# QiaoK/MPI-Asynchronous-Communication-Test

Measured on AMD Instinct MI355X. Metric: aggregate exchange GB/s + max total time, all-to-many/many-to-all, 1–8 GPUs, higher is better.
Workload: dtype u8

## Files before the change

### include/xg.h

```cpp
#ifndef XG_H
#define XG_H

#include <stddef.h>
#include <stdint.h>

#include "xg_sched.h"

#ifdef __cplusplus
extern "C" {
#endif

#define XG_OK 0
#define XG_EHIP 1
#define XG_ERCCL 2
#define XG_EARG 3
#define XG_ENOMEM 4

#define XG_UNIQUE_ID_BYTES 128

typedef struct xg_ctx xg_ctx;
typedef struct xg_regions xg_regions;
typedef struct xg_plan xg_plan;

int xg_get_unique_id(void *uid );
// ... 29 lines not shown
int xg_chk_spans(xg_regions *r, const xg_bufspan *spans, int n, uint64_t *chk);

int xg_plan_load(xg_ctx *ctx, xg_regions *r, const xg_devplan *dp, xg_plan **out);
int xg_plan_free(xg_plan *p);
int xg_plan_nsteps(const xg_plan *p);
int xg_plan_run(xg_plan *p, double *step_done, double *step_post, double *wall);
int xg_plan_enqueue(xg_plan *p);
int xg_plan_check(xg_plan *p);
int xg_plan_engine(const xg_plan *p);
int xg_plan_engine_rails(const xg_plan *p);
int xg_plan_engine_steps(const xg_plan *p, int *nseg, int *nhaz);
int xg_plan_launches(const xg_plan *p);
int xg_plan_wave_launches(const xg_plan *p, int *grid, int *max_pieces_per_wave);
int xg_plan_shift_launches(const xg_plan *p);
int xg_plan_extent_launches(const xg_plan *p);
int xg_plan_displs(const xg_plan *p, int64_t *out, int n);
int xg_vplans_run(xg_plan *const *plans, int n, double *step_done);
int xg_vplans_run_rccl(xg_plan *const *plans, int n, double *step_done);
int xg_plan_set_local_only(xg_plan *p, int on);
int xg_plan_set_step_marks(xg_plan *p, const uint8_t *need);
int xg_ktime_begin(xg_ctx *ctx, int max_launches, int mode);
int xg_ktime_end(xg_ctx *ctx, double *total_ms, int *launches, int64_t *bytes);
int xg_ktime_launch(xg_ctx *ctx, int k, double *ms, int64_t *bytes);

int xg_p2p_bench(xg_ctx *ctx, int64_t bytes, int mode, int reps, double *gbps, double *sec);
int xg_p2p_split_bench(xg_ctx *ctx, int64_t bytes, int calls, int reps, double *gbps, double *sec);
int xg_p2p_pair_bench(xg_ctx *ctx, int64_t bytes, int peer, int reps, double *gbps, double *sec);

int xg_set_copy_params(xg_ctx *ctx, int64_t chunk_bytes, int variant);

// ... 65 lines not shown
```

### include/xg_sched.h

```cpp
#ifndef XG_SCHED_H
#define XG_SCHED_H

#include <stddef.h>
#include <stdint.h>

#ifdef __cplusplus
extern "C" {
#endif

typedef struct {
    double post_request_time;
    double send_wait_all_time;
    double recv_wait_all_time;
    double barrier_time;
    double total_time;
} xg_timer;

enum { XG_A2M = 0, XG_M2A = 1 };

typedef struct {
    int32_t src, sseg, dst, dslot;
    int64_t len;
    int32_t step;
    int32_t flags;
// ... 130 lines not shown
#define XG_SOLO_OFF_MAX (1ull << 24)
#define XG_SOLO_WIDE_OFF_MAX (1ull << 32)
typedef struct { int32_t rails, npieces, nrows, nmeta; } xg_solo_shape;
int xg_solo_tables(const xg_span *xfer, const int *step_begin, int nsteps, int rails_max, int waves,
                   uint64_t src_base, uint64_t dst_base, xg_solo_shape *shape, uint64_t *descs, int *meta);
#define XG_SOLO_BEFORE_SHIFT(g) ((g) == 16 ? 55 : (g) == 4 ? 57 : 59)
int xg_solo_tables_g(const xg_span *xfer, const int *step_begin, int nsteps, int rails_max, int waves, int granule,
                     uint64_t src_base, uint64_t dst_base, xg_solo_shape *shape, uint64_t *descs, int *meta);
void xg_solo_reduce_stamps(const uint64_t *stamps, int rails, int64_t stride, int s0, int s1, uint64_t *out);

int64_t xg_piece_size(const int64_t *lens, int n, int64_t chunk, int cus, int64_t wg_cost);
int xg_step_local_meets_unpacks(const xg_devplan *dp, int s);
int xg_step_stage_meets_rest(const xg_devplan *dp, int s);
int xg_extent_tiles(const int64_t *lens, int n, int64_t tile_bytes, int tile_pieces, int32_t *begin);

typedef struct { int32_t rank, agg; int64_t off, len; } xg_ext;
int xg_exts_lens(const xg_ext *exts, int64_t n, int procs, int cb_nodes, int64_t *lens);
int xg_exts_check(const xg_ext *exts, int64_t n, int procs, int cb_nodes, const int64_t *dom_bytes, int scatter,
                  char *err, size_t errlen);
int64_t xg_domain_offset(const xg_sched *s, int ngpus, int a, const int64_t *dom_bytes);
int64_t xg_domain_bytes(const xg_sched *s, int ngpus, int g, const int64_t *dom_bytes);
xg_devplan *xg_place_plan_build(const xg_sched *s, int ngpus, int g, const xg_ext *exts, int64_t n,
                                const int64_t *dom_bytes);

typedef struct { int32_t rank, seed0; int64_t off; int32_t nsegs, pad; } xg_segrun;
typedef struct { int32_t src, seed, dst, pad; int64_t off; } xg_slot;

enum { XG_FP_REFERENCE = 0, XG_FP_STRONG = 1 };

int xg_fill_runs(const xg_sched *s, int ngpus, int g, xg_segrun *out);
// ... 17 lines not shown
```

### mpi-asynchronous-communication-test_amd/csrc/host/pieces.c

```c
#include "xg_sched.h"

#include <stdlib.h>

int64_t xg_piece_size(const int64_t *lens, int n, int64_t chunk, int cus, int64_t wg_cost)
{
    int64_t best_c = chunk, cand;
    double best = -1;
    int i;
    if (!lens || n <= 0 || chunk <= 0 || cus <= 0) return chunk;
    for (cand = chunk; cand >= 4096 && (cand & 15) == 0; cand /= 2) {
        int64_t w = 0;
        double cost;
        for (i = 0; i < n; ++i)
            if (lens[i] > 0) w += (lens[i] + cand - 1) / cand;
        if (!w) return chunk;
        cost = (double)((w + cus - 1) / cus) * (double)(cand + wg_cost);
        if (best < 0 || cost < best) {
            best = cost;
            best_c = cand;
        }
    }
    return best_c;
}

// ... 7 lines not shown
        return 0;
    }
    for (i = 0; i < n; ++i) {
        const int64_t l = lens[i] > 0 ? lens[i] : 0;
        if (cnt && (cnt >= tile_pieces || bytes + l > tile_bytes)) cnt = 0;
        if (!cnt) {
            if (begin) begin[nt] = i;
            ++nt;
            bytes = 0;
        }
        ++cnt;
        bytes += l;
    }
    if (begin) begin[nt] = n;
    return nt;
}

typedef struct { int64_t lo, hi; } ival;

static int ival_cmp(const void *x, const void *y)
{
    const ival *a = (const ival *)x, *b = (const ival *)y;
    return a->lo < b->lo ? -1 : a->lo > b->lo;
}

int xg_step_local_meets_unpacks(const xg_devplan *dp, int s)
{
    const xg_stepplan *pv, *sp;
    ival *w[XG_NBUF] = {0};
    int64_t *reach[XG_NBUF] = {0};
// ... 120 lines not shown
```

### mpi-asynchronous-communication-test_amd/csrc/kernels.h

```cpp
#pragma once
#include <hip/hip_runtime.h>
#include <stdint.h>
#include <type_traits>

namespace xgk {

constexpr int kThreads = 256;

struct DCopy {
    const uint8_t *src;
    uint8_t *dst;
    int64_t len;
};

struct DSeg {
    int64_t off;
    int32_t rank, seed;
};

struct DSlot {
    int64_t off;
    int32_t src, seed;
};

// ... 248 lines not shown
    load(a, pa);
    for (int k = 0;; k += 2) {
        if (k + 1 < n) {
            pb = next(k + 1);
            load(b, pb);
        }
        store(a, pa);
        if (k + 1 >= n) break;
        if (k + 2 < n) {
            pa = next(k + 2);
            load(a, pa);
        }
        store(b, pb);
        if (k + 2 >= n) break;
    }
}

[[maybe_unused]] static __global__ void clock_kernel(unsigned long long *t)
{
    if (threadIdx.x == 0) *t = (unsigned long long)wall_clock64();
}

struct EngineState {
    unsigned count;
    unsigned tmo;
    unsigned rails;
    unsigned arrive;
    unsigned pad[4];
    unsigned go[16][32];
    unsigned fin[16][32];
// ... 775 lines not shown
```

### mpi-asynchronous-communication-test_amd/csrc/runtime/ctx.hip

```cpp
#include "rt.h"

#include <dirent.h>
#include <limits.h>
#include <link.h>

#include <string>

extern "C" double xg_now(void)
{
    struct timespec ts;
    clock_gettime(CLOCK_MONOTONIC, &ts);
    return ts.tv_sec + ts.tv_nsec * 1e-9;
}

static void share_gpu_env(int rank)
{
    const char *v = getenv("XG_SHARE_GPU");
    if (!v || strcmp(v, "1")) return;
    char id[64];
    snprintf(id, sizeof id, "xg-share-gpu-rank-%d", rank);
    setenv("NCCL_HOSTID", id, 1);
    setenv("NCCL_SOCKET_IFNAME", "lo", 0);
    setenv("NCCL_MAX_NCHANNELS", "2", 0);
}
// ... 143 lines not shown
    (void)rank;
    c->chunk = 32768; c->variant = 0; c->kt_mode = 0; c->nk = 0; c->kt_bytes = 0;
    const char *env = getenv("XG_COPY_VARIANT");
    if (env && (atoi(env) == 1 || atoi(env) == 6)) c->variant = atoi(env);
    else if (env && atoi(env) != 0) fprintf(stderr, "xg: XG_COPY_VARIANT=%s ignored (0, 1 or 6)\n", env);
    env = getenv("XG_RAGGED_COPY");
    c->ragged_copy = !(env && atoi(env) == 0);
    env = getenv("XG_EXTENT_COPY");
    c->extent_copy = env ? atoi(env) != 0 : kExtDefault;
    c->extent_mean_max = kExtMeanMax;
    env = getenv("XG_EXTENT_MEAN_MAX");
    if (env && atol(env) > 0) c->extent_mean_max = atol(env);
    c->extent_tile = kExtTileBytes;
    env = getenv("XG_EXTENT_TILE_KIB");
    if (env && atoi(env) > 0 && atoi(env) <= 1024) c->extent_tile = (int64_t)atoi(env) << 10;
    c->engine_max_step = 16 << 20;
    env = getenv("XG_ENGINE_MAX_STEP");
    if (env) c->engine_max_step = atol(env);
    {
        int cus = 0, per_cu = 0;
        HIPCHK(hipDeviceGetAttribute(&cus, hipDeviceAttributeMultiprocessorCount, device));
        HIPCHK(hipOccupancyMaxActiveBlocksPerMultiprocessor(&per_cu, xgk::step_engine_kernel<16>, xgk::kThreads, 0));
        c->engine_occ = cus * (per_cu < 1 ? 1 : per_cu);
        c->engine_wmax = cus;
        if (c->engine_wmax > c->engine_occ) c->engine_wmax = c->engine_occ;
        if (c->engine_wmax < 1) c->engine_wmax = 1;
    }
    env = getenv("XG_ENGINE_DRAIN");
    c->engine_drain = env && !strcmp(env, "1");
    env = getenv("XG_ENGINE_SOLO");
// ... 391 lines not shown
```

### mpi-asynchronous-communication-test_amd/csrc/runtime/exec.hip

```cpp
#include "rt.h"

extern "C" const char *xg_debug_where(void)
{
    static char buf[160];
    snprintf(buf, sizeof buf, "%s: step %d of %d: %s", g_where.fn, g_where.step, g_where.nsteps, g_where.phase);
    return buf;
}


int mark(xg_plan *p, int i, hipStream_t stream)
{
    hipLaunchKernelGGL(xgk::clock_kernel, dim3(1), dim3(64), 0, stream, p->d_gstamp + i + 1);
    HIPCHK(hipGetLastError());
    return XG_OK;
}

int read_marks(const xg_plan *p, std::vector<unsigned long long> &gs)
{
    gs.resize((size_t)p->nsteps + 1);
    HIPCHK(hipMemcpy(gs.data(), p->d_gstamp, 8 * gs.size(), hipMemcpyDeviceToHost));
    return XG_OK;
}

double mark_elapsed(const xg_plan *p, int i, const std::vector<unsigned long long> &gs)
{
    return (double)(gs[i + 1] - gs[0]) / p->ctx->wall_hz;
}


static int wave_wgs(const xg_plan *p, int n) { return std::max(1, std::min(p->ctx->wave_grid, (n + 3) / 4)); }

static int launch_one(xg_plan *p, const CopyLaunch &l, int b, int n, hipStream_t st, unsigned long long *start)
{
    const xgk::DCopy *pc = p->d_pieces + b;
    if (l.kib && b == l.b) {
        const auto k = l.kib == 2   ? xgk::copy_kernel_w<2>
                       : l.kib == 4 ? xgk::copy_kernel_w<4>
                                    : xgk::copy_kernel_w<xgk::kWaveKiB>;
        hipLaunchKernelGGL(k, dim3(wave_wgs(p, n)), dim3(xgk::kThreads), 0, st, pc, n, start);
    } else if (l.ext) {
        int k = 0;
        while (k + 1 < l.ndisp && p->cuts[l.cut + k + 1] <= b) ++k;
        const auto kx = l.nt ? xgk::copy_kernel_x<true> : xgk::copy_kernel_x<false>;
        hipLaunchKernelGGL(kx, dim3(p->xt_n[l.xt + k]), dim3(xgk::kThreads), 0, st, pc, p->d_xt + p->xt_off[l.xt + k],
                           start);
    } else if (l.shift) {
        const auto k = l.nt ? xgk::copy_kernel_s<true> : xgk::copy_kernel_s<false>;
        hipLaunchKernelGGL(k, dim3(n), dim3(xgk::kThreads), 0, st, pc, start);
    } else {
        const auto k = l.nt ? xgk::copy_kernel_g<4, true> : xgk::copy_kernel_g<4>;
// ... 17 lines not shown
        c->kbytes[c->nk] = 2 * bytes;
    }
    if (kt || c->kt_mode == 2) {
        c->nk++;
        c->kt_bytes += 2 * bytes;
    }
    return XG_OK;
}

static int launch_copy(xg_plan *p, const CopyLaunch &l, hipStream_t st, unsigned long long *start)
{
    if (start && !l.stamps) return XG_EARG;
    const int *cut = p->cuts.data() + l.cut;
    int rc;
    for (int k = 0; k < l.ndisp; ++k) {
        const int64_t nb = l.ndisp == 1 ? l.bytes : p->plen[cut[k + 1]] - p->plen[cut[k]];
        bool kt;
        if ((rc = kt_before(p->ctx, st, &kt))) return rc;
        if ((rc = launch_one(p, l, cut[k], cut[k + 1] - cut[k], st, k == 0 ? start : nullptr))) return rc;
        if ((rc = kt_after(p->ctx, st, kt, nb))) return rc;
    }
    return XG_OK;
}

int enqueue_pre(xg_plan *p, int s, hipStream_t stream, hipStream_t side, unsigned long long *start)
{
    const StepR &st = p->steps[s];
    int rc;
    for (int i = st.l_b; i < st.l_rccl; ++i) {
        const CopyLaunch &l = p->launches[i];
        if (l.side) {
// ... 24 lines not shown
    each_launch(p, [&](const CopyLaunch &l) {
        if (!l.kib) return;
        const int m = p->cuts[l.cut + 1] - l.b, w = wave_wgs(p, m);
        ++count;
        most = std::max(most, (m + 4 * w - 1) / (4 * w));
    });
    if (grid) *grid = p->ctx->wave_grid;
    if (max_pieces_per_wave) *max_pieces_per_wave = most;
    return count;
}

extern "C" int xg_plan_shift_launches(const xg_plan *p)
{
    int count = 0;
    each_launch(p, [&](const CopyLaunch &l) { count += l.shift; });
    return count;
}

extern "C" int xg_plan_extent_launches(const xg_plan *p)
{
    int count = 0;
    each_launch(p, [&](const CopyLaunch &l) { count += l.ext; });
    return count;
}

static int enqueue_step(xg_plan *p, int s)
{
    xg_ctx *c = p->ctx;
    const StepR &st = p->steps[s];
    int rc;
// ... 315 lines not shown
```

### mpi-asynchronous-communication-test_amd/csrc/runtime/plan_load.hip

```cpp
#include "rt.h"

static uint64_t next_plan_id()
{
    static uint64_t n = 0;
    return __atomic_add_fetch(&n, 1, __ATOMIC_RELAXED);
}

static bool engine_step(const xg_ctx *c, const StepR &st)
{
    return !st.p2p_n && !st.sync_after && !st.stage_n && !st.stage_fused && !st.post_n && !st.pack_n && !st.fused &&
           !st.deferred && st.local_bytes <= c->engine_max_step;
}

static_assert(xgk::kSoloWaves == XG_SOLO_WAVES && xgk::kSoloMaxRails == XG_SOLO_MAX_RAILS &&
                  xgk::kSoloPiece == XG_SOLO_PIECE && xgk::kSoloK == XG_SOLO_K &&
                  xgk::kSoloMaxSteps == XG_SOLO_MAX_STEPS && xgk::kSoloMaxPieces == XG_SOLO_MAX_PIECES &&
                  xgk::kSoloOffMax == XG_SOLO_OFF_MAX && xgk::kSoloWideOffMax == XG_SOLO_WIDE_OFF_MAX,
              "solo engine constants: kernels.h and xg_sched.h disagree");

static bool solo_pays(int64_t bytes, int n, int rails, int wv, int busy, int gran = 16)
{
    const double traffic = 2.0 * (double)bytes;
    const double rail = 15e9 * gran / 16.0;
    const double solo = wv == 1 ? traffic / std::min(rails * rail, 6e12 * gran / 16.0) + n * 0.05e-6
                                : traffic / (rails * 120e9) + n * 0.2e-6;
    const double grid = traffic / 5e12 + n * 1.0e-6 + (busy < 2 ? 8e-6 : 0.0);
// ... 386 lines not shown
    typedef std::pair<int, int> Range;
    xg_plan *p;
    const xg_devplan *dp;
    std::vector<xgk::DCopy> &pieces;
    DisplScan &ds;
    int64_t chunk = 0;
    CopyLaunch *cur = nullptr;

    int64_t bytes_of(Range rg) const
    {
        int64_t n = 0;
        for (int i = 0; i < rg.second; ++i) n += std::max<int64_t>(0, dp->copies[rg.first + i].len);
        return n;
    }

    void open(CopyLaunch &l, std::initializer_list<Range> ranges, bool cross, bool reread_cut, bool reread_run)
    {
        const xg_ctx *c = p->ctx;
        cur = &l;
        l.b = (int)pieces.size();
        chunk = c->chunk;
        uint64_t bits = 0;
        std::vector<int64_t> lens;
        for (const Range &rg : ranges)
            for (int i = 0; i < rg.second; ++i) {
                const xg_copy &cp = dp->copies[rg.first + i];
                lens.push_back(cp.len);
                if (cp.len <= 0) continue;
                l.bytes += cp.len;
                bits |= (uint64_t)cp.src_off | (uint64_t)cp.dst_off | (uint64_t)cp.len;
            }
// ... 3 lines not shown
        l.stamps = v == 1 || v == 6;
        l.shift = (dp->flags & XG_DP_RAGGED) && c->ragged_copy && (bits & 15) != 0;
        int64_t npos = 0;
        for (int64_t n : lens) npos += n > 0;
        l.ext = (dp->flags & XG_DP_EXTENTS) && c->extent_copy && l.stamps && c->chunk <= (1 << 24) &&
                l.bytes <= npos * c->extent_mean_max;
        if (l.ext) l.shift = false;
        if (!l.ext && cross && l.bytes >= c->wave_min && l.bytes <= kWaveMax && (bits & 15) == 0 &&
            copy_variant(p, l.bytes, reread_cut) == 1) {
            const int kib = c->wave_kib ? c->wave_kib : wave_kib_for(l.bytes, c->cus);
            chunk = (int64_t)kib << 10;
            if (v == 1) l.kib = kib;
        } else {
            chunk = xg_piece_size(lens.data(), (int)lens.size(), c->chunk, c->cus, kWgCost);
        }
    }
    void close() { cur->n = (int)pieces.size() - cur->b; }

    bool add(const xg_copy &cp, int side)
    {
        const xg_regions *r = p->reg;
        if (cp.len <= 0) return true;
        if (cp.src_buf < 0 || cp.src_buf >= XG_NBUF || cp.dst_buf < 0 || cp.dst_buf >= XG_NBUF) return false;
        if (cp.src_off < 0 || cp.dst_off < 0 || cp.src_off + cp.len > r->bytes[cp.src_buf] ||
            cp.dst_off + cp.len > r->bytes[cp.dst_buf])
            return false;
        const int ci = (int)ds.len.size();
        if (side >= 0) {
            ds.len.push_back(cp.len);
            ds.host.push_back(side == 0 ? cp.dst_off : cp.src_off);
        }
        for (int64_t o = 0; o < cp.len; o += chunk) {
            xgk::DCopy d;
            d.src = r->ptr[cp.src_buf] + (side == 1 ? 0 : cp.src_off) + o;
            d.dst = r->ptr[cp.dst_buf] + (side == 0 ? 0 : cp.dst_off) + o;
            d.len = cp.len - o < chunk ? cp.len - o : chunk;
            if (side >= 0) ds.fix.push_back({(int)pieces.size(), ci, o, side, 0});
            pieces.push_back(d);
        }
        return true;
    }
// ... 43 lines not shown
        st.stage_b = (int)pieces.size();
        if (st.stage_fused) {
            open(local, {r_stage, r_local, r_pack}, cross, true, true);
            if (!add_range(r_stage, -1)) return false;
        } else {
            open(stage, {r_stage}, false, true, true);
            if (!add_range(r_stage, -1)) return false;
            close();
            st.stage_n = stage.n;
            st.stage_bytes = stage.bytes;
            if (st.fused_local) {
                open(local, {r_prev, r_local, r_pack}, true, true, true);
                local.mark_prev = true;
                if (!add_post(s - 1)) return false;
            } else if (st.split) {
                open(local, {r_local}, true, false, false);
                local.side = true;
            } else if (!st.fused) {
                open(local, {r_local, r_pack}, cross, r_pack.second > 0, bytes_of(r_pack) > 0);
            }
        }
        st.local_b = st.stage_fused ? st.stage_b : (int)pieces.size();
        if (!add_range(r_local, -1)) return false;
        st.local_n = (int)pieces.size() - st.local_b;
        st.local_bytes = span(st.local_b);
        if (st.split || (st.fused && !st.fused_local)) {
            if (st.split) close();
            open(pack, {r_prev, r_pack}, true, true, true);
            pack.mark_prev = st.fused;
            if (st.fused && !add_post(s - 1)) return false;
        }
        st.pack_b = (int)pieces.size();
        if (!add_range(r_pack, 0)) return false;
        ds.close_group();
        st.pack_n = (int)pieces.size() - st.pack_b;
        st.pack_bytes = span(st.pack_b);
        st.pre_n = st.local_n + st.pack_n;
        close();
        st.post_b = (int)pieces.size();
        if (!st.deferred) {
            open(post, {r_post}, true, false, false);
            if (!add_post(s)) return false;
            close();
        }
        std::vector<CopyLaunch> &tab = p->launches;
        auto push = [&](const CopyLaunch &l) {
            if (l.n > 0) tab.push_back(l);
        };
        const bool pack_first = st.fused || c->split_after_pack;
        st.l_b = (int)tab.size();
        push(stage);
        if (pack_first) push(pack);
        push(local);
        if (!pack_first) push(pack);
        st.l_rccl = (int)tab.size();
        push(post);
        st.l_e = (int)tab.size();
        return true;
    }
};

static bool build_tables(xg_plan *p, const xg_devplan *dp, std::vector<xgk::DCopy> &pieces, DisplScan &ds)
// ... 14 lines not shown
    for (const StepR &st : p->steps) {
        if (st.post_n < 2) continue;
        std::vector<int> idx(st.post_n);
        for (int i = 0; i < st.post_n; ++i) idx[i] = st.post_b + i;
        std::stable_sort(idx.begin(), idx.end(), [&](int x, int y) { return pieces[x].dst < pieces[y].dst; });
        std::vector<xgk::DCopy> sorted(st.post_n);
        for (int i = 0; i < st.post_n; ++i) sorted[i] = pieces[idx[i]];
        for (int i = 0; i < st.post_n; ++i) {
            const int f = where[idx[i]];
            if (f >= 0) ds.fix[f].piece = st.post_b + i;
        }
        std::copy(sorted.begin(), sorted.end(), pieces.begin() + st.post_b);
    }
}

static void cut_launches(xg_plan *p)
{
    const int64_t cap = p->ctx->launch_max;
    const int64_t *pre = p->plen.data();
    for (CopyLaunch &l : p->launches) {
        const int end = l.b + l.n;
        l.cut = (int)p->cuts.size();
        p->cuts.push_back(l.b);
        for (int o = l.b; cap > 0 && l.bytes > cap + cap / 2 && o < end;) {
            int e = (int)(std::lower_bound(pre + o + 1, pre + end + 1, pre[o] + cap) - pre);
            if (e > end) e = end;
            if (end - e < 16 || pre[end] - pre[e] < cap / 2) e = end;
            if (e < end) p->cuts.push_back(e);
            o = e;
        }
        p->cuts.push_back(end);
        l.ndisp = (int)p->cuts.size() - 1 - l.cut;
    }
}

// ... 41 lines not shown
            p->chain_end[s] = e;
            any = true;
        }
        s = e > s ? e : s + 1;
    }
    return any;
}

static int plan_upload(xg_plan *p, const std::vector<xgk::DCopy> &pieces, DisplScan &ds)
{
    int rc;
    if (p->npieces) {
        HIPCHK(hipMalloc(&p->d_pieces, sizeof(xgk::DCopy) * pieces.size()));
        HIPCHK(hipMemcpy(p->d_pieces, pieces.data(), sizeof(xgk::DCopy) * pieces.size(), hipMemcpyHostToDevice));
    }
    if (!p->xt_begin.empty()) {
        HIPCHK(hipMalloc(&p->d_xt, sizeof(int) * p->xt_begin.size()));
        HIPCHK(hipMemcpy(p->d_xt, p->xt_begin.data(), sizeof(int) * p->xt_begin.size(), hipMemcpyHostToDevice));
    }
    p->need_mark.assign(p->nsteps, 1);
    p->fork.assign(p->nsteps, nullptr);
    p->join.assign(p->nsteps, nullptr);
    for (int s = 0; s < p->nsteps; ++s)
        for (int i = p->steps[s].l_b; i < p->steps[s].l_rccl; ++i)
            if (p->launches[i].side) {
                HIPCHK(hipEventCreateWithFlags(&p->fork[s], hipEventDisableTiming));
                HIPCHK(hipEventCreateWithFlags(&p->join[s], hipEventDisableTiming));
            }
    HIPCHK(hipMalloc(&p->d_gstamp, 8 * ((size_t)p->nsteps + 1)));
    if ((rc = run_displ_scan(p, ds)) || (rc = build_segments(p, pieces))) return rc;
// ... 47 lines not shown
    p->graph_auto = c->nranks == 1 && !c->virt && run <= ((int64_t)16 << 20);
    *out = p;
    return XG_OK;
}

extern "C" int xg_plan_free(xg_plan *p)
{
    if (!p) return XG_OK;
    hipError_t first = hipSuccess;
    auto keep = [&](hipError_t e) {
        if (e != hipSuccess && first == hipSuccess) first = e;
    };
    keep(hipStreamSynchronize(p->ctx->stream));
    keep(hipStreamSynchronize(p->ctx->side));
    for (void *q : {(void *)p->d_pieces, (void *)p->d_sb, (void *)p->d_epieces, (void *)p->d_engine,
                    (void *)p->d_disp, (void *)p->d_solo, (void *)p->d_cstamp, (void *)p->d_gstamp, (void *)p->d_xt})
        if (q) keep(hipFree(q));
    if (p->db) keep(hipHostFree((void *)p->db));
    for (auto &e : p->fork) if (e) keep(hipEventDestroy(e));
    for (auto &e : p->join) if (e) keep(hipEventDestroy(e));
    for (hipGraphExec_t g : {p->g_enq, p->g_run, p->vg.exec})
        if (g) keep(hipGraphExecDestroy(g));
    delete p;
    if (first != hipSuccess) {
        fprintf(stderr, "xg: HIP error %s while freeing a plan\n", hipGetErrorString(first));
        return XG_EHIP;
    }
    return XG_OK;
}

extern "C" int xg_plan_nsteps(const xg_plan *p) { return p->nsteps; }
// ... 30 lines not shown
```

### mpi-asynchronous-communication-test_amd/csrc/runtime/rt.h

```cpp
#pragma once

#include <hip/hip_runtime.h>
#include <unistd.h>
#include <rccl/rccl.h>

#include <stdio.h>
#include <stdlib.h>
#include <string.h>
#include <time.h>

#include <algorithm>
#include <vector>

#include "../kernels.h"
#include "xg.h"

#define HIPCHK(x)                                                                                  \
    do {                                                                                           \
        hipError_t e_ = (x);                                                                       \
        if (e_ != hipSuccess) {                                                                    \
            fprintf(stderr, "xg: HIP error %s at %s:%d: %s\n", hipGetErrorString(e_), __FILE__,   \
                    __LINE__, #x);                                                                 \
            (void)hipGetLastError();                                                               \
            return XG_EHIP;                                                                        \
// ... 88 lines not shown
    int cus;
    int step_chain;
    int engine_arm;
    int64_t split_min;
    int64_t self_max;
    int fuse_stage;
    int split_after_pack;
    int graph;
    double wall_hz;
    int variant;
    int ragged_copy;
    int extent_copy;
    int64_t extent_mean_max;
    int64_t extent_tile;
    int engine_occ;
    int kt_mode;
    int nk;
    std::vector<hipEvent_t> kev;
    std::vector<int64_t> kbytes;
    int64_t kt_bytes;
};

struct xg_regions {
    xg_ctx *ctx;
    uint8_t *ptr[XG_NBUF];
    int64_t bytes[XG_NBUF];
    bool owned[XG_NBUF];
};

struct CopyLaunch {
    int b = 0, n = 0;
    int64_t bytes = 0;
    int kib = 0;
    bool nt = false;
    bool shift = false;
    bool ext = false;
    int xt = 0;
    bool stamps = false;
    bool side = false;
    bool mark_prev = false;
    int cut = 0, ndisp = 1;
};

struct StepR {
    int stage_b = 0, stage_n = 0, local_b = 0, local_n = 0, pack_b = 0, pack_n = 0, post_b = 0, post_n = 0;
    int call_b = 0, call_n = 0, p2p_n = 0, sync_after = 0;
    int groups = 1;
    int posts = 0;
    int pre_n = 0;
    int64_t stage_bytes = 0, local_bytes = 0, pack_bytes = 0, post_bytes = 0;
    bool split = false, fused = false, deferred = false;
    bool self_local = false;
    bool fused_local = false;
    bool stage_fused = false;
    int l_b = 0, l_rccl = 0, l_e = 0;
};

struct EngSeg {
    int s0, s1;
    int w, b;
    int sb_off;
    int nhaz;
    bool solo;
    int wv;
    int gran;
    int u0;
// ... 4 lines not shown
};

struct xg_plan {
    xg_ctx *ctx = nullptr;
    xg_regions *reg = nullptr;
    int nsteps = 0;
    xgk::DCopy *d_pieces = nullptr;
    int npieces = 0;
    std::vector<StepR> steps;
    std::vector<xg_call> calls;
    std::vector<int32_t> call_begin;
    std::vector<CopyLaunch> launches;
    std::vector<int> cuts;
    std::vector<int> xt_begin, xt_off, xt_n;
    int *d_xt = nullptr;
    std::vector<hipEvent_t> fork, join;
    int variant = 0;
    bool streaming = false;
    std::vector<int> seg_of;
    std::vector<EngSeg> segs;
    int *d_sb = nullptr;
    xgk::DCopy *d_epieces = nullptr;
    xgk::EngineState *d_engine = nullptr;
    int stamp_rails = 1;
    unsigned engine_base = 0;
    bool engine_reset = false;
    xgk::Doorbell *db = nullptr;
    std::vector<unsigned long long> solo_desc;
    unsigned long long *d_solo = nullptr;
    unsigned epoch = 0;
// ... 44 lines not shown
        *out = nullptr;
        fprintf(stderr, "xg: hipGraphInstantiate: %s\n", hipGetErrorString(ie));
        return XG_EHIP;
    }
    return XG_OK;
}

constexpr int64_t kNtMin = 128 << 20;
constexpr int64_t kNtStream = 4 << 20;
constexpr int64_t kGridCacheMax = 256 << 20;
constexpr int64_t kWgCost = 2048;
constexpr int64_t kExtTileBytes = 32 << 10;
constexpr int kExtTilePieces = xgk::kThreads;
constexpr int64_t kExtMeanMax = 1024;
constexpr int kExtDefault = 1;
constexpr int64_t kWaveMax = 32 << 20;
static inline int wave_kib_for(int64_t bytes, int cus)
{
    for (int kib = 8; kib > 2; kib /= 2)
        if (bytes / ((int64_t)kib << 10) >= 4 * (int64_t)cus) return kib;
    return 2;
}

static inline void rccl_log_to_stderr()
{
    if (!getenv("NCCL_DEBUG_FILE")) setenv("NCCL_DEBUG_FILE", "/dev/stderr", 0);
}

struct StdoutToStderr {
    int saved;
// ... 24 lines not shown
```

### mpi-asynchronous-communication-test_amd/xg.py

```python
import ctypes as C
import os

HERE = os.path.dirname(os.path.abspath(__file__))
LIBDIR = os.environ.get("XG_LIBDIR") or os.path.join(HERE, "lib")


class XGError(RuntimeError):
    pass


class Timer(C.Structure):
    _fields_ = [("post_request_time", C.c_double), ("send_wait_all_time", C.c_double),
                ("recv_wait_all_time", C.c_double), ("barrier_time", C.c_double),
                ("total_time", C.c_double)]

    def as_tuple(self):
        return (self.post_request_time, self.send_wait_all_time, self.recv_wait_all_time,
                self.barrier_time, self.total_time)


NBUF = 5


class Msg(C.Structure):
# ... 151 lines not shown
        h.xg_devplan_build_form.argtypes = [C.c_void_p, C.c_int, C.c_int, C.c_int64, C.c_int64, C.c_int]
        h.xg_devplan_free.argtypes = [C.POINTER(DevPlan)]
        h.xg_devplan_step_calls.argtypes = [C.POINTER(DevPlan), C.c_int, C.c_int64, C.POINTER(Call)]
        h.xg_devplan_step_self_calls.argtypes = [C.POINTER(DevPlan), C.c_int, C.c_int64]
        h.xg_calls_match.restype = C.c_int64
        h.xg_calls_match.argtypes = [C.c_int, C.c_int, C.POINTER(C.POINTER(Call)), C.POINTER(C.POINTER(C.c_int32)),
                                     C.POINTER(CallPair), C.c_int64, C.c_char_p, C.c_size_t]
        h.xg_devplans_match.restype = C.c_int64
        h.xg_devplans_match.argtypes = [C.POINTER(C.POINTER(DevPlan)), C.c_int, C.c_int64, C.POINTER(CallPair),
                                        C.c_int64, C.c_char_p, C.c_size_t]
        h.xg_step_local_meets_unpacks.argtypes = [C.POINTER(DevPlan), C.c_int]
        h.xg_step_stage_meets_rest.argtypes = [C.POINTER(DevPlan), C.c_int]
        h.xg_piece_size.restype = C.c_int64
        h.xg_piece_size.argtypes = [C.POINTER(C.c_int64), C.c_int, C.c_int64, C.c_int, C.c_int64]
        h.xg_extent_tiles.argtypes = [C.POINTER(C.c_int64), C.c_int, C.c_int64, C.c_int, C.POINTER(C.c_int32)]
        h.xg_exts_lens.argtypes = [C.POINTER(Ext), C.c_int64, C.c_int, C.c_int, C.POINTER(C.c_int64)]
        h.xg_exts_check.argtypes = [C.POINTER(Ext), C.c_int64, C.c_int, C.c_int, C.POINTER(C.c_int64), C.c_int,
                                    C.c_char_p, C.c_size_t]
        h.xg_domain_offset.restype = C.c_int64
        h.xg_domain_offset.argtypes = [C.c_void_p, C.c_int, C.c_int, C.POINTER(C.c_int64)]
        h.xg_domain_bytes.restype = C.c_int64
        h.xg_domain_bytes.argtypes = [C.c_void_p, C.c_int, C.c_int, C.POINTER(C.c_int64)]
        h.xg_place_plan_build.restype = C.POINTER(DevPlan)
        h.xg_place_plan_build.argtypes = [C.c_void_p, C.c_int, C.c_int, C.POINTER(Ext), C.c_int64, C.POINTER(C.c_int64)]
        h.xg_fill_runs.argtypes = [C.c_void_p, C.c_int, C.c_int, C.POINTER(SegRun)]
        h.xg_verify_slots.argtypes = [C.c_void_p, C.c_int, C.c_int, C.POINTER(Slot)]
        h.xg_deliveries.argtypes = [C.c_void_p, C.c_int, C.POINTER(Delivery)]
        h.xg_engine_hazards.argtypes = [C.POINTER(Span), C.POINTER(C.c_int), C.c_int, C.c_int, C.POINTER(C.c_int)]
        h.xg_solo_reduce_stamps.argtypes = [C.POINTER(C.c_uint64), C.c_int, C.c_int64, C.c_int, C.c_int,
                                            C.POINTER(C.c_uint64)]
# ... 103 lines not shown

def piece_size(lens, chunk=32768, cus=256, wg_cost=2048):
    arr = (C.c_int64 * max(1, len(lens)))(*lens)
    return host().xg_piece_size(arr, len(lens), chunk, cus, wg_cost)


def extent_tiles(lens, tile_bytes=32768, tile_pieces=256):
    n = len(lens)
    arr = (C.c_int64 * max(1, n))(*lens)
    nt = host().xg_extent_tiles(arr, n, tile_bytes, tile_pieces, None)
    if nt < 0:
        return None
    begin = (C.c_int32 * (nt + 1))()
    assert host().xg_extent_tiles(arr, n, tile_bytes, tile_pieces, begin) == nt
    return list(begin)


def _ext_array(exts):
    v = [e if isinstance(e, Ext) else Ext(*[int(x) for x in e]) for e in exts]
    return (Ext * max(1, len(v)))(*v), len(v)


def exts_lens(exts, procs, cb_nodes):
    arr, n = _ext_array(exts)
    out = (C.c_int64 * (procs * cb_nodes))()
    if host().xg_exts_lens(arr, n, procs, cb_nodes, out) != 0:
        raise XGError("xg_exts_lens: rank or aggregator out of range, negative length or overflow")
    return list(out)


# ... 302 lines not shown
        d.xg_verify.argtypes = [vp, C.POINTER(Slot), ip, i64, ip, ip, C.POINTER(C.c_uint64),
                                C.POINTER(i64), C.POINTER(i64)]
        d.xg_plan_load.argtypes = [vp, vp, C.POINTER(DevPlan), C.POINTER(vp)]
        d.xg_plan_free.argtypes = [vp]
        d.xg_plan_nsteps.argtypes = [vp]
        d.xg_plan_run.argtypes = [vp, C.POINTER(C.c_double), C.POINTER(C.c_double), C.POINTER(C.c_double)]
        d.xg_plan_enqueue.argtypes = [vp]
        d.xg_plan_engine.argtypes = [vp]
        d.xg_plan_engine_rails.argtypes = [vp]
        d.xg_plan_check.argtypes = [vp]
        d.xg_plan_launches.argtypes = [vp]
        d.xg_plan_engine_steps.argtypes = [vp, C.POINTER(ip), C.POINTER(ip)]
        d.xg_plan_wave_launches.argtypes = [vp, C.POINTER(ip), C.POINTER(ip)]
        d.xg_plan_shift_launches.argtypes = [vp]
        d.xg_plan_extent_launches.argtypes = [vp]
        d.xg_exchange_w.argtypes = [vp, ip, ip, ip, C.POINTER(Ext), i64, C.POINTER(i64), C.POINTER(ip), ip, vp, vp,
                                    C.POINTER(Timer), ip, ip, C.POINTER(RunOpts), C.POINTER(i64), C.POINTER(i64),
                                    C.POINTER(C.c_double), C.c_char_p, C.c_size_t]
        d.xg_plan_displs.argtypes = [vp, C.POINTER(i64), ip]
        d.xg_ktime_begin.argtypes = [vp, ip, ip]
        d.xg_ktime_end.argtypes = [vp, C.POINTER(C.c_double), C.POINTER(ip), C.POINTER(i64)]
        d.xg_ktime_launch.argtypes = [vp, ip, C.POINTER(C.c_double), C.POINTER(i64)]
        d.xg_set_copy_params.argtypes = [vp, i64, ip]
        d.xg_p2p_bench.argtypes = [vp, i64, ip, ip, C.POINTER(C.c_double), C.POINTER(C.c_double)]
        d.xg_p2p_pair_bench.argtypes = [vp, i64, ip, ip, C.POINTER(C.c_double), C.POINTER(C.c_double)]
        d.xg_p2p_split_bench.argtypes = [vp, i64, ip, ip, C.POINTER(C.c_double), C.POINTER(C.c_double)]
        d.xg_rccl_version.argtypes = [C.POINTER(C.c_int)]
        _dev = d
    return _dev

# ... 411 lines not shown
```

### profiles/copy_ceiling.py

```python
import ctypes as C
import os

HERE = os.path.dirname(os.path.dirname(os.path.abspath(__file__)))
lib = C.CDLL(os.path.join(HERE, "mpi-asynchronous-communication-test_amd", "tools", "lib", "libxgtools.so"))
lib.xgt_copy_ceiling.argtypes = [C.c_int, C.c_int64, C.c_int, C.c_int, C.POINTER(C.c_double)]
names = {0: "grid-stride copy", 1: "copy_kernel_g<4> 32K", 2: "copy_kernel_b<4,sc1>", 3: "read-only", 4: "write-only",
         5: "hipMemcpy DtoD", 6: "grid-stride copy nt", 7: "copy_kernel_g<4> 256K", 8: "copy_kernel_g<4> 64K",
         9: "copy_kernel_g<4,nt> 32K", 10: "read-only nt", 11: "write-only nt", 12: "grid-stride nt-load",
         13: "grid-stride nt-store", 14: "copy_kernel_g<8,nt> 32K", 15: "copy_kernel_g<2,nt> 32K",
         16: "m2a gather 32M stride", 17: "m2a gather skewed", 18: "c2 pack g<4> 16K", 19: "c2 pack p<4> x512",
         20: "c2 pack p<2> x512", 21: "c2 pack p<8> x256", 22: "c2 pack w<8> 8K", 23: "m2a gather w<8,nt> 8K",
         24: "m2a gather w<4,nt> 4K", 25: "m2a gather w<16,nt> 16K", 26: "c2 pack2 g<4> 16K", 27: "c2 pack2 w<8> 8K",
         28: "m2a g<4,nt> 64K", 29: "m2a g<8,nt> 32K", 30: "m2a g<4,nt> 128K", 31: "m2a g<4,nt> 16K",
         32: "m2a bb ld nt st nt", 33: "m2a bb ld nt st nt|sc1", 34: "m2a bb nt|sc0|sc1 both",
         35: "m2a bb ld nt st sc0|sc1", 36: "m2a bb ld plain st nt", 37: "m2a bb ld nt st plain",
         38: "contig bb ld nt st nt|sc1", 39: "m2a bb nt|sc1 both"}
kinds = [int(k) for k in os.environ.get("KINDS", "0,1,2,3,4,5,6,7,8,9").split(",")]
sizes = [int(x) << 20 for x in os.environ.get("SIZES_MIB", "448,1024,4096").split(",")]
for nb in sizes:
    for kind in kinds:
        g = C.c_double()
        assert lib.xgt_copy_ceiling(0, nb, kind, 20, C.byref(g)) == 0
        print("bytes=%d %-22s %.1f GB/s" % (nb, names[kind], g.value), flush=True)
```

Before: 3040.

## Add small-piece copy kernel that indexes uniform copies arithmetically per block

Adds a copy_kernel_q path for local steps whose copies all have the same length. Each block computes its copy index and offset arithmetically, interleaving k copies per group sorted by destination, so no per-piece descriptor table is needed. It is enabled by default for steps of at least 112 MiB and excludes those steps from the engine path. The aim is finer 4/8 KiB work units and less descriptor overhead, at the cost of many more small blocks and a different launch split.

```diff
diff --git a/include/xg.h b/include/xg.h
--- a/include/xg.h
+++ b/include/xg.h
@@ -67,6 +67,7 @@
 int xg_plan_wave_launches(const xg_plan *p, int *grid, int *max_pieces_per_wave);
 int xg_plan_shift_launches(const xg_plan *p);
 int xg_plan_extent_launches(const xg_plan *p);
+int xg_plan_small_launches(const xg_plan *p, int *kib);
 int xg_plan_displs(const xg_plan *p, int64_t *out, int n);
 int xg_vplans_run(xg_plan *const *plans, int n, double *step_done);
 int xg_vplans_run_rccl(xg_plan *const *plans, int n, double *step_done);
diff --git a/include/xg_sched.h b/include/xg_sched.h
--- a/include/xg_sched.h
+++ b/include/xg_sched.h
@@ -168,6 +168,28 @@
 int xg_step_stage_meets_rest(const xg_devplan *dp, int s);
 int xg_extent_tiles(const int64_t *lens, int n, int64_t tile_bytes, int tile_pieces, int32_t *begin);
 
+#if defined(__HIPCC__)
+#define XG_HD __host__ __device__
+#else
+#define XG_HD
+#endif
+typedef struct { uint32_t copy; int64_t off, n; } xg_small_at;
+inline XG_HD uint32_t xg_small_ppc(int64_t len, int64_t piece) { return (uint32_t)((len + piece - 1) / piece); }
+inline XG_HD xg_small_at xg_small_index(uint32_t b, uint32_t copies, int64_t len, int64_t piece, uint32_t k)
+{
+    const uint32_t gs = k * xg_small_ppc(len, piece);
+    const uint32_t g = b / gs, r = b - g * gs;
+    const uint32_t left = copies - g * k, kk = left < k ? left : k;
+    const uint32_t j = r / kk;
+    xg_small_at a;
+    a.copy = g * k + (r - j * kk);
+    a.off = (int64_t)j * piece;
+    a.n = len - a.off < piece ? len - a.off : piece;
+    return a;
+}
+int xg_small_piece_at(int64_t b, int64_t copies, int64_t len, int64_t piece, int k, int64_t *copy, int64_t *off,
+                      int64_t *n);
+
 typedef struct { int32_t rank, agg; int64_t off, len; } xg_ext;
 int xg_exts_lens(const xg_ext *exts, int64_t n, int procs, int cb_nodes, int64_t *lens);
 int xg_exts_check(const xg_ext *exts, int64_t n, int procs, int cb_nodes, const int64_t *dom_bytes, int scatter,
diff --git a/mpi-asynchronous-communication-test_amd/csrc/host/pieces.c b/mpi-asynchronous-communication-test_amd/csrc/host/pieces.c
--- a/mpi-asynchronous-communication-test_amd/csrc/host/pieces.c
+++ b/mpi-asynchronous-communication-test_amd/csrc/host/pieces.c
@@ -45,6 +45,24 @@
     }
     if (begin) begin[nt] = n;
     return nt;
+}
+
+extern inline uint32_t xg_small_ppc(int64_t len, int64_t piece);
+extern inline xg_small_at xg_small_index(uint32_t b, uint32_t copies, int64_t len, int64_t piece, uint32_t k);
+
+int xg_small_piece_at(int64_t b, int64_t copies, int64_t len, int64_t piece, int k, int64_t *copy, int64_t *off,
+                      int64_t *n)
+{
+    xg_small_at a;
+    if (b < 0 || copies < 1 || len < 1 || piece < 1 || k < 1 || k > (1 << 20)) return -1;
+    if (copies * (int64_t)xg_small_ppc(len, piece) > INT32_MAX || (int64_t)k * xg_small_ppc(len, piece) > INT32_MAX ||
+        b >= copies * (int64_t)xg_small_ppc(len, piece))
+        return -1;
+    a = xg_small_index((uint32_t)b, (uint32_t)copies, len, piece, (uint32_t)k);
+    if (copy) *copy = a.copy;
+    if (off) *off = a.off;
+    if (n) *n = a.n;
+    return 0;
 }
 
 typedef struct { int64_t lo, hi; } ival;
diff --git a/mpi-asynchronous-communication-test_amd/csrc/kernels.h b/mpi-asynchronous-communication-test_amd/csrc/kernels.h
--- a/mpi-asynchronous-communication-test_amd/csrc/kernels.h
+++ b/mpi-asynchronous-communication-test_amd/csrc/kernels.h
@@ -2,6 +2,8 @@
 #include <hip/hip_runtime.h>
 #include <stdint.h>
 #include <type_traits>
+
+#include "../../include/xg_sched.h"
 
 namespace xgk {
 
@@ -286,6 +288,24 @@
         store(b, pb);
         if (k + 2 >= n) break;
     }
+}
+
+template <int L, bool NT = false>
+__global__ __launch_bounds__(kThreads) void copy_kernel_q(const DCopy *__restrict__ rows, uint32_t base,
+                                                          uint32_t copies, int64_t len, uint32_t k,
+                                                          unsigned long long *start)
+{
+    constexpr int AUX = NT ? kAuxNT : kAuxPlain;
+    if (start && blockIdx.x == 0 && threadIdx.x == 0) *start = (unsigned long long)wall_clock64();
+    const xg_small_at a = xg_small_index(base + blockIdx.x, copies, len, (int64_t)L * kTile, k);
+    const DCopy c = rows[__builtin_amdgcn_readfirstlane((int)a.copy)];
+    const brsrc rs = make_rsrc(c.src + a.off, a.n), rd = make_rsrc(c.dst + a.off, a.n);
+    const int o = (int)threadIdx.x * 16;
+    u32x4 v[L];
+#pragma unroll
+    for (int j = 0; j < L; ++j) v[j] = bload16a<AUX>(rs, o + j * kTile);
+#pragma unroll
+    for (int j = 0; j < L; ++j) bstore16<AUX>(rd, o + j * kTile, v[j]);
 }
 
 [[maybe_unused]] static __global__ void clock_kernel(unsigned long long *t)
diff --git a/mpi-asynchronous-communication-test_amd/csrc/runtime/ctx.hip b/mpi-asynchronous-communication-test_amd/csrc/runtime/ctx.hip
--- a/mpi-asynchronous-communication-test_amd/csrc/runtime/ctx.hip
+++ b/mpi-asynchronous-communication-test_amd/csrc/runtime/ctx.hip
@@ -181,6 +181,17 @@
     c->extent_tile = kExtTileBytes;
     env = getenv("XG_EXTENT_TILE_KIB");
     if (env && atoi(env) > 0 && atoi(env) <= 1024) c->extent_tile = (int64_t)atoi(env) << 10;
+    env = getenv("XG_SMALL_PIECES");
+    c->small_pieces = env ? atoi(env) != 0 : kSmallDefault;
+    c->small_piece_min = kSmallMin;
+    env = getenv("XG_SMALL_PIECE_MIN");
+    if (env && atoll(env) >= 0) c->small_piece_min = atoll(env);
+    c->small_kib = kSmallKiB;
+    env = getenv("XG_SMALL_PIECE_KIB");
+    if (env && (atoi(env) == 4 || atoi(env) == 8)) c->small_kib = atoi(env);
+    c->small_order = kSmallOrder;
+    env = getenv("XG_SMALL_PIECE_ORDER");
+    if (env && atoi(env) >= 1 && atoi(env) <= 1024) c->small_order = atoi(env);
     c->engine_max_step = 16 << 20;
     env = getenv("XG_ENGINE_MAX_STEP");
     if (env) c->engine_max_step = atol(env);
diff --git a/mpi-asynchronous-communication-test_amd/csrc/runtime/exec.hip b/mpi-asynchronous-communication-test_amd/csrc/runtime/exec.hip
--- a/mpi-asynchronous-communication-test_amd/csrc/runtime/exec.hip
+++ b/mpi-asynchronous-communication-test_amd/csrc/runtime/exec.hip
@@ -33,7 +33,12 @@
 static int launch_one(xg_plan *p, const CopyLaunch &l, int b, int n, hipStream_t st, unsigned long long *start)
 {
     const xgk::DCopy *pc = p->d_pieces + b;
-    if (l.kib && b == l.b) {
+    if (l.q) {
+        const auto k = l.q == 1 ? (l.nt ? xgk::copy_kernel_q<1, true> : xgk::copy_kernel_q<1, false>)
+                                : (l.nt ? xgk::copy_kernel_q<2, true> : xgk::copy_kernel_q<2, false>);
+        hipLaunchKernelGGL(k, dim3(n), dim3(xgk::kThreads), 0, st, p->d_rows + l.q_row, (uint32_t)b,
+                           (uint32_t)l.q_copies, l.q_len, (uint32_t)l.q_k, start);
+    } else if (l.kib && b == l.b) {
         const auto k = l.kib == 2   ? xgk::copy_kernel_w<2>
                        : l.kib == 4 ? xgk::copy_kernel_w<4>
                                     : xgk::copy_kernel_w<xgk::kWaveKiB>;
@@ -81,7 +86,7 @@
     const int *cut = p->cuts.data() + l.cut;
     int rc;
     for (int k = 0; k < l.ndisp; ++k) {
-        const int64_t nb = l.ndisp == 1 ? l.bytes : p->plen[cut[k + 1]] - p->plen[cut[k]];
+        const int64_t nb = l.q ? p->qbytes[l.q_bytes + k] : l.ndisp == 1 ? l.bytes : p->plen[cut[k + 1]] - p->plen[cut[k]];
         bool kt;
         if ((rc = kt_before(p->ctx, st, &kt))) return rc;
         if ((rc = launch_one(p, l, cut[k], cut[k + 1] - cut[k], st, k == 0 ? start : nullptr))) return rc;
@@ -136,6 +141,17 @@
 {
     int count = 0;
     each_launch(p, [&](const CopyLaunch &l) { count += l.shift; });
+    return count;
+}
+
+extern "C" int xg_plan_small_launches(const xg_plan *p, int *kib)
+{
+    int count = 0, q = 0;
+    each_launch(p, [&](const CopyLaunch &l) {
+        count += l.q != 0;
+        if (l.q) q = l.q;
+    });
+    if (kib) *kib = 4 * q;
     return count;
 }
 
diff --git a/mpi-asynchronous-communication-test_amd/csrc/runtime/plan_load.hip b/mpi-asynchronous-communication-test_amd/csrc/runtime/plan_load.hip
--- a/mpi-asynchronous-communication-test_amd/csrc/runtime/plan_load.hip
+++ b/mpi-asynchronous-communication-test_amd/csrc/runtime/plan_load.hip
@@ -9,7 +9,7 @@
 static bool engine_step(const xg_ctx *c, const StepR &st)
 {
     return !st.p2p_n && !st.sync_after && !st.stage_n && !st.stage_fused && !st.post_n && !st.pack_n && !st.fused &&
-           !st.deferred && st.local_bytes <= c->engine_max_step;
+           !st.deferred && !st.small && st.local_bytes <= c->engine_max_step;
 }
 
 static_assert(xgk::kSoloWaves == XG_SOLO_WAVES && xgk::kSoloMaxRails == XG_SOLO_MAX_RAILS &&
@@ -426,7 +426,8 @@
         return n;
     }
 
-    void open(CopyLaunch &l, std::initializer_list<Range> ranges, bool cross, bool reread_cut, bool reread_run)
+    void open(CopyLaunch &l, std::initializer_list<Range> ranges, bool cross, bool reread_cut, bool reread_run,
+              bool may_small = false)
     {
         const xg_ctx *c = p->ctx;
         cur = &l;
@@ -460,8 +461,35 @@
         } else {
             chunk = xg_piece_size(lens.data(), (int)lens.size(), c->chunk, c->cus, kWgCost);
         }
-    }
-    void close() { cur->n = (int)pieces.size() - cur->b; }
+        if (!may_small || !c->small_pieces || l.ext || l.shift || l.kib || !l.stamps || (bits & 15) != 0 ||
+            l.bytes < c->small_piece_min)
+            return;
+        int64_t len = 0;
+        bool uniform = true;
+        for (const Range &rg : ranges)
+            for (int i = 0; i < rg.second; ++i) {
+                const xg_copy &cp = dp->copies[rg.first + i];
+                if (cp.len <= 0) continue;
+                uniform = uniform && (len == 0 || cp.len == len) && cp.dst_buf != XG_BUF_STAGE_SEND &&
+                          cp.src_buf != XG_BUF_STAGE_RECV;
+                len = cp.len;
+            }
+        const int64_t piece = (int64_t)c->small_kib << 10;
+        const int64_t ppc = (len + piece - 1) / piece;
+        if (!uniform || npos * ppc > INT32_MAX || c->small_order * ppc > INT32_MAX) return;
+        l.q = c->small_kib / 4;
+        l.q_len = len;
+        l.q_k = c->small_order;
+        l.q_row = (int)p->rows.size();
+    }
+    void close()
+    {
+        cur->n = (int)pieces.size() - cur->b;
+        if (!cur->q) return;
+        cur->q_copies = (int)p->rows.size() - cur->q_row;
+        std::stable_sort(p->rows.begin() + cur->q_row, p->rows.end(),
+                         [](const xgk::DCopy &x, const xgk::DCopy &y) { return x.dst < y.dst; });
+    }
 
     bool add(const xg_copy &cp, int side)
     {
@@ -471,6 +499,10 @@
         if (cp.src_off < 0 || cp.dst_off < 0 || cp.src_off + cp.len > r->bytes[cp.src_buf] ||
             cp.dst_off + cp.len > r->bytes[cp.dst_buf])
             return false;
+        if (cur->q) {
+            p->rows.push_back({r->ptr[cp.src_buf] + cp.src_off, r->ptr[cp.dst_buf] + cp.dst_off, cp.len});
+            return side < 0;
+        }
         const int ci = (int)ds.len.size();
         if (side >= 0) {
             ds.len.push_back(cp.len);
@@ -544,16 +576,20 @@
                 local.mark_prev = true;
                 if (!add_post(s - 1)) return false;
             } else if (st.split) {
-                open(local, {r_local}, true, false, false);
+                open(local, {r_local}, true, false, false, true);
                 local.side = true;
             } else if (!st.fused) {
-                open(local, {r_local, r_pack}, cross, r_pack.second > 0, bytes_of(r_pack) > 0);
+                open(local, {r_local, r_pack}, cross, r_pack.second > 0, bytes_of(r_pack) > 0, true);
             }
         }
         st.local_b = st.stage_fused ? st.stage_b : (int)pieces.size();
         if (!add_range(r_local, -1)) return false;
         st.local_n = (int)pieces.size() - st.local_b;
         st.local_bytes = span(st.local_b);
+        if (local.q) {
+            st.small = true;
+            st.local_bytes = local.bytes;
+        }
         if (st.split || (st.fused && !st.fused_local)) {
             if (st.split) close();
             open(pack, {r_prev, r_pack}, true, true, true);
@@ -575,7 +611,7 @@
         }
         std::vector<CopyLaunch> &tab = p->launches;
         auto push = [&](const CopyLaunch &l) {
-            if (l.n > 0) tab.push_back(l);
+            if (l.n > 0 || l.q) tab.push_back(l);
         };
         const bool pack_first = st.fused || c->split_after_pack;
         st.l_b = (int)tab.size();
@@ -620,11 +656,36 @@
     }
 }
 
+static void cut_small(xg_plan *p, CopyLaunch &l)
+{
+    const int64_t cap = p->ctx->launch_max, piece = (int64_t)l.q * xgk::kTile;
+    const int64_t W = (int64_t)l.q_copies * xg_small_ppc(l.q_len, piece);
+    l.cut = (int)p->cuts.size();
+    p->cuts.push_back(0);
+    if (cap > 0 && l.bytes > cap + cap / 2) {
+        const int64_t per = std::max<int64_t>(1, cap / piece);
+        for (int64_t o = per; o < W && (W - o) * piece >= cap / 2 && W - o >= 16; o += per) p->cuts.push_back((int)o);
+    }
+    p->cuts.push_back((int)W);
+    l.ndisp = (int)p->cuts.size() - 1 - l.cut;
+    l.q_bytes = (int)p->qbytes.size();
+    for (int k = 0; k < l.ndisp; ++k) {
+        int64_t nb = 0;
+        for (int64_t b = p->cuts[l.cut + k]; b < p->cuts[l.cut + k + 1]; ++b)
+            nb += xg_small_index((uint32_t)b, (uint32_t)l.q_copies, l.q_len, piece, (uint32_t)l.q_k).n;
+        p->qbytes.push_back(nb);
+    }
+}
+
 static void cut_launches(xg_plan *p)
 {
     const int64_t cap = p->ctx->launch_max;
     const int64_t *pre = p->plen.data();
     for (CopyLaunch &l : p->launches) {
+        if (l.q) {
+            cut_small(p, l);
+            continue;
+        }
         const int end = l.b + l.n;
         l.cut = (int)p->cuts.size();
         p->cuts.push_back(l.b);
@@ -696,6 +757,10 @@
         HIPCHK(hipMalloc(&p->d_pieces, sizeof(xgk::DCopy) * pieces.size()));
         HIPCHK(hipMemcpy(p->d_pieces, pieces.data(), sizeof(xgk::DCopy) * pieces.size(), hipMemcpyHostToDevice));
     }
+    if (!p->rows.empty()) {
+        HIPCHK(hipMalloc(&p->d_rows, sizeof(xgk::DCopy) * p->rows.size()));
+        HIPCHK(hipMemcpy(p->d_rows, p->rows.data(), sizeof(xgk::DCopy) * p->rows.size(), hipMemcpyHostToDevice));
+    }
     if (!p->xt_begin.empty()) {
         HIPCHK(hipMalloc(&p->d_xt, sizeof(int) * p->xt_begin.size()));
         HIPCHK(hipMemcpy(p->d_xt, p->xt_begin.data(), sizeof(int) * p->xt_begin.size(), hipMemcpyHostToDevice));
@@ -773,7 +838,8 @@
     keep(hipStreamSynchronize(p->ctx->stream));
     keep(hipStreamSynchronize(p->ctx->side));
     for (void *q : {(void *)p->d_pieces, (void *)p->d_sb, (void *)p->d_epieces, (void *)p->d_engine,
-                    (void *)p->d_disp, (void *)p->d_solo, (void *)p->d_cstamp, (void *)p->d_gstamp, (void *)p->d_xt})
+                    (void *)p->d_disp, (void *)p->d_solo, (void *)p->d_cstamp, (void *)p->d_gstamp, (void *)p->d_xt,
+                    (void *)p->d_rows})
         if (q) keep(hipFree(q));
     if (p->db) keep(hipHostFree((void *)p->db));
     for (auto &e : p->fork) if (e) keep(hipEventDestroy(e));
diff --git a/mpi-asynchronous-communication-test_amd/csrc/runtime/rt.h b/mpi-asynchronous-communication-test_amd/csrc/runtime/rt.h
--- a/mpi-asynchronous-communication-test_amd/csrc/runtime/rt.h
+++ b/mpi-asynchronous-communication-test_amd/csrc/runtime/rt.h
@@ -126,6 +126,10 @@
     int64_t extent_mean_max;
     int64_t extent_tile;
     int engine_occ;
+    int small_pieces;
+    int64_t small_piece_min;
+    int small_kib;
+    int small_order;
     int kt_mode;
     int nk;
     std::vector<hipEvent_t> kev;
@@ -148,6 +152,9 @@
     bool shift = false;
     bool ext = false;
     int xt = 0;
+    int q = 0;
+    int q_row = 0, q_copies = 0, q_k = 1, q_bytes = 0;
+    int64_t q_len = 0;
     bool stamps = false;
     bool side = false;
     bool mark_prev = false;
@@ -162,6 +169,7 @@
     int pre_n = 0;
     int64_t stage_bytes = 0, local_bytes = 0, pack_bytes = 0, post_bytes = 0;
     bool split = false, fused = false, deferred = false;
+    bool small = false;
     bool self_local = false;
     bool fused_local = false;
     bool stage_fused = false;
@@ -196,6 +204,9 @@
     std::vector<int> cuts;
     std::vector<int> xt_begin, xt_off, xt_n;
     int *d_xt = nullptr;
+    std::vector<xgk::DCopy> rows;
+    xgk::DCopy *d_rows = nullptr;
+    std::vector<int64_t> qbytes;
     std::vector<hipEvent_t> fork, join;
     int variant = 0;
     bool streaming = false;
@@ -270,6 +281,10 @@
 constexpr int kExtTilePieces = xgk::kThreads;
 constexpr int64_t kExtMeanMax = 1024;
 constexpr int kExtDefault = 1;
+constexpr int64_t kSmallMin = 112 << 20;
+constexpr int kSmallKiB = 8;
+constexpr int kSmallOrder = 8;
+constexpr int kSmallDefault = 1;
 constexpr int64_t kWaveMax = 32 << 20;
 static inline int wave_kib_for(int64_t bytes, int cus)
 {
diff --git a/mpi-asynchronous-communication-test_amd/xg.py b/mpi-asynchronous-communication-test_amd/xg.py
--- a/mpi-asynchronous-communication-test_amd/xg.py
+++ b/mpi-asynchronous-communication-test_amd/xg.py
@@ -189,6 +189,7 @@
         h.xg_piece_size.restype = C.c_int64
         h.xg_piece_size.argtypes = [C.POINTER(C.c_int64), C.c_int, C.c_int64, C.c_int, C.c_int64]
         h.xg_extent_tiles.argtypes = [C.POINTER(C.c_int64), C.c_int, C.c_int64, C.c_int, C.POINTER(C.c_int32)]
+        h.xg_small_piece_at.argtypes = [C.c_int64, C.c_int64, C.c_int64, C.c_int64, C.c_int] + [C.POINTER(C.c_int64)] * 3
         h.xg_exts_lens.argtypes = [C.POINTER(Ext), C.c_int64, C.c_int, C.c_int, C.POINTER(C.c_int64)]
         h.xg_exts_check.argtypes = [C.POINTER(Ext), C.c_int64, C.c_int, C.c_int, C.POINTER(C.c_int64), C.c_int,
                                     C.c_char_p, C.c_size_t]
@@ -322,6 +323,13 @@
     begin = (C.c_int32 * (nt + 1))()
     assert host().xg_extent_tiles(arr, n, tile_bytes, tile_pieces, begin) == nt
     return list(begin)
+
+
+def small_piece_at(b, copies, length, piece, k=1):
+    out = [C.c_int64() for _ in range(3)]
+    if host().xg_small_piece_at(b, copies, length, piece, k, *[C.byref(x) for x in out]) != 0:
+        return None
+    return tuple(x.value for x in out)
 
 
 def _ext_array(exts):
@@ -654,6 +662,7 @@
         d.xg_plan_wave_launches.argtypes = [vp, C.POINTER(ip), C.POINTER(ip)]
         d.xg_plan_shift_launches.argtypes = [vp]
         d.xg_plan_extent_launches.argtypes = [vp]
+        d.xg_plan_small_launches.argtypes = [vp, C.POINTER(ip)]
         d.xg_exchange_w.argtypes = [vp, ip, ip, ip, C.POINTER(Ext), i64, C.POINTER(i64), C.POINTER(ip), ip, vp, vp,
                                     C.POINTER(Timer), ip, ip, C.POINTER(RunOpts), C.POINTER(i64), C.POINTER(i64),
                                     C.POINTER(C.c_double), C.c_char_p, C.c_size_t]
diff --git a/profiles/copy_ceiling.py b/profiles/copy_ceiling.py
--- a/profiles/copy_ceiling.py
+++ b/profiles/copy_ceiling.py
@@ -14,7 +14,9 @@
          28: "m2a g<4,nt> 64K", 29: "m2a g<8,nt> 32K", 30: "m2a g<4,nt> 128K", 31: "m2a g<4,nt> 16K",
          32: "m2a bb ld nt st nt", 33: "m2a bb ld nt st nt|sc1", 34: "m2a bb nt|sc0|sc1 both",
          35: "m2a bb ld nt st sc0|sc1", 36: "m2a bb ld plain st nt", 37: "m2a bb ld nt st plain",
-         38: "contig bb ld nt st nt|sc1", 39: "m2a bb nt|sc1 both"}
+         38: "contig bb ld nt st nt|sc1", 39: "m2a bb nt|sc1 both", 40: "contig q<1,nt> 4K k1", 41: "contig q<2,nt> 8K k1",
+         42: "contig q<2,nt> 8K k8", 43: "m2a q<1,nt> 4K k1", 44: "m2a q<2,nt> 8K k1", 45: "m2a q<2,nt> 8K k8",
+         46: "m2a q<1,nt> 4K k8"}
 kinds = [int(k) for k in os.environ.get("KINDS", "0,1,2,3,4,5,6,7,8,9").split(",")]
 sizes = [int(x) << 20 for x in os.environ.get("SIZES_MIB", "448,1024,4096").split(",")]
 for nb in sizes:
diff --git a/profiles/small_pieces_summary.py b/profiles/small_pieces_summary.py
--- /dev/null
+++ b/profiles/small_pieces_summary.py
@@ -0,0 +1,56 @@
+#!/usr/bin/env python3
+import csv
+import os
+import statistics
+import sys
+
+
+def pct(v, q):
+    v = sorted(v)
+    return v[min(len(v) - 1, int(q * len(v)))]
+
+
+def runs(files):
+    arms = {}
+    for f in files:
+        name = os.path.basename(f).rsplit(".", 1)[0]
+        rows = [tuple(float(x) for x in line.split()[:3]) for line in open(f) if line.strip()]
+        arms[name] = rows
+        for i, r in enumerate(rows):
+            print("%-16s run %d: %8.2f GB/s  %.4f ms per step  %.2f us per launch" % ((name, i + 1) + r))
+    st = {}
+    for name, rows in arms.items():
+        ms = [r[1] for r in rows]
+        st[name] = (statistics.median(ms), min(ms), max(ms))
+        print("%-16s median %.4f ms per step (min %.4f max %.4f, spread %.4f), median %.2f GB/s"
+              % (name, st[name][0], st[name][1], st[name][2], st[name][2] - st[name][1],
+                 statistics.median(r[0] for r in rows)))
+    base = os.path.basename(files[0]).rsplit(".", 1)[0]
+    bm, blo, bhi = st[base]
+    for name, (m, lo, hi) in st.items():
+        if name == base:
+            continue
+        need = max(bhi - blo, hi - lo)
+        print("%s vs %s: median %+.4f ms (%+.2f %%), larger spread %.4f ms -> %s"
+              % (name, base, m - bm, (m - bm) / bm * 100, need,
+                 "wins by the rule" if bm - m > need else "does not win by the rule"))
+
+
+def trace(path, steps=50):
+    rows = [r for r in csv.DictReader(open(path)) if "copy_kernel" in r["Kernel_Name"]]
+    rows.sort(key=lambda r: int(r["Start_Timestamp"]))
+    rows = rows[-4 * steps:] if len(rows) >= 4 * steps else rows[len(rows) % 4:]
+    name = rows[0]["Kernel_Name"].split("(")[0].replace("void ", "").replace("xgk::", "")
+    print("%d launches of %s, grid %s" % (len(rows), name, rows[0]["Grid_Size_X"]))
+    tot = 0.0
+    for p in range(4):
+        us = [(int(r["End_Timestamp"]) - int(r["Start_Timestamp"])) / 1e3 for r in rows[p::4]]
+        tot += statistics.mean(us)
+        print("position %d: mean %.2f us  median %.2f  p10 %.2f  p90 %.2f  (%d launches)"
+              % (p + 1, statistics.mean(us), statistics.median(us), pct(us, 0.1), pct(us, 0.9), len(us)))
+    gaps = [(int(b["Start_Timestamp"]) - int(a["End_Timestamp"])) / 1e3 for a, b in zip(rows, rows[1:])]
+    print("sum of the four means %.2f us per step; gap between launches: mean %.2f us" % (tot, statistics.mean(gaps)))
+
+
+if __name__ == "__main__":
+    {"runs": runs, "trace": lambda a: trace(a[0])}[sys.argv[1]](sys.argv[2:])
```

Measured after the change: 3171, median of 6. 1.04x the previous value.
